# pymc-devs/pymc

Measured on AMD Instinct MI355X. Metric: effective samples/sec (and leapfrog steps/sec), 10k-param hierarchical logistic regression, one NUTS chain per GPU, higher is better.
Workload: dtype f64

## Files before the change

include/nuts_mi355.h:

```cpp
#ifndef NUTS_MI355_H
#define NUTS_MI355_H

#include <stdint.h>

#ifdef __cplusplus
extern "C" {
#endif

#define NUTS_OK 0
#define NUTS_E_BAD_ENERGY 1
#define NUTS_E_ARG 2
#define NUTS_E_HIP 3
#define NUTS_E_LINALG 4
#define NUTS_E_CALLBACK 5


enum { NUTS_TR_NONE = 0, NUTS_TR_LOG = 1, NUTS_TR_LOGODDS = 2, NUTS_TR_INTERVAL = 3 };
enum {
  NUTS_OP_CONST = 0, NUTS_OP_DATA = 1, NUTS_OP_VAR = 2,
  NUTS_OP_TMP = 3,
  NUTS_OP_GATHER = 4,
  NUTS_OP_LIN = 5
};
enum {
// ... 117 lines not shown
  const double *mix_w_const;
  const double *mix_w_alpha;
  int64_t glm_N;
  int32_t glm_P, glm_family, glm_beta, glm_intercept, glm_sigma, glm_beta_derived;
  double glm_sigma_const;
  const double *glm_X;
  const double *glm_y;
  int32_t n_lins, pad3;
  const nuts_lin *lins;
} nuts_model_spec;
enum { NUTS_GLM_NORMAL = 0, NUTS_GLM_BERNOULLI = 1, NUTS_GLM_POISSON = 2 };
#define NUTS_GLM_MAXP 512

typedef struct nuts_model nuts_model;
typedef struct nuts_chain nuts_chain;

int nuts_set_option(const char *name, int32_t value);
int nuts_unset_option(const char *name);
void nuts_clear_options(void);

int64_t nuts_edge_pair_plan(const int32_t *dirs, int32_t n_dirs, int32_t n_doublings, int32_t spec, int32_t max_depth,
                            int32_t ring, int32_t *out, int64_t out_cap);

int nuts_device_count(void);
int nuts_set_device(int device);
const char *nuts_last_error(void);

nuts_model *nuts_model_create(const nuts_model_spec *spec);
void nuts_model_destroy(nuts_model *m);
int32_t nuts_model_ndim(const nuts_model *m);
int nuts_model_logp_grad(nuts_model *m, const double *q, double *logp, double *grad);
int nuts_model_time_logp_grad(nuts_model *m, const double *q, int reps, double *ms_total, double *ms_dominant);
int nuts_model_debug_ticks(nuts_model *m, int64_t *out );
int64_t nuts_model_algorithmic_bytes(const nuts_model *m);
int nuts_model_get_scalar(const nuts_model *m, const char *name, double *out);

enum { NUTS_LL_FACTOR = 0, NUTS_LL_LOGIT_ROWS = 1, NUTS_LL_MIXTURE = 2, NUTS_LL_GLM = 3 };
int nuts_model_loglik_size(nuts_model *m, int32_t kind, int32_t index, int64_t *n);
int nuts_model_loglik(nuts_model *m, int32_t kind, int32_t index, const double *q, int64_t S, double *out);
typedef struct nuts_waic nuts_waic;
nuts_waic *nuts_waic_create(nuts_model *m, int32_t kind, int32_t index);
int nuts_waic_update(nuts_waic *w, const double *q, int64_t S);
int nuts_waic_read(nuts_waic *w, double *lppd_i, double *p_waic_i, int64_t *n_draws);
int nuts_waic_read_raw(nuts_waic *w, double *acc);
void nuts_waic_destroy(nuts_waic *w);
typedef struct nuts_psis nuts_psis;
// ... 193 lines not shown
```

pymc_amd/_lib.py:

```python

from __future__ import annotations

import ctypes as C
import os
import threading

import numpy as np

_HERE = os.path.dirname(os.path.abspath(__file__))
LIB_PATH = os.path.join(_HERE, "libnuts_mi355.so")

NUTS_OK, NUTS_E_BAD_ENERGY, NUTS_E_ARG, NUTS_E_HIP, NUTS_E_LINALG, NUTS_E_CALLBACK = 0, 1, 2, 3, 4, 5


class EngineError(RuntimeError):
    """A HIP/runtime failure inside libnuts_mi355 (maps to ParallelSamplingError-style reporting)."""


class Operand(C.Structure):
    _fields_ = [("kind", C.c_int32), ("ref", C.c_int32), ("c", C.c_double)]


class Term(C.Structure):
    _fields_ = [("a", Operand), ("b", Operand), ("c", Operand)]
# ... 215 lines not shown
    "nuts_chain_get_scalar": (C.c_int, [_VP, C.c_char_p, _PD]),
    "nuts_chain_get_vector": (C.c_int, [_VP, C.c_char_p, _PD]),
    "nuts_chain_set_dense": (C.c_int, [_VP, _PD, _PD]),
    "nuts_chain_set_diag": (C.c_int, [_VP, _PD, _PD, _PD]),
    "nuts_chain_set_host_potential": (C.c_int, [_VP, VelocityFn, EnergyFn, VelocityEnergyFn, _VP]),
    "nuts_chain_welford_export": (C.c_int, [_VP, _VP]),
    "nuts_chain_welford_import": (C.c_int, [_VP, _VP]),
    "nuts_chain_set_log_step_bar": (C.c_int, [_VP, C.c_double, C.c_double]),
    "nuts_gibbs_plan": (C.c_int, [C.POINTER(Pcg64), C.c_int64, C.c_int32, _VP, _VP, _VP, _PD]),
    "nuts_gibbs_plan_shuffle": (C.c_int, [C.POINTER(Pcg64), C.c_int64, _VP]),
    "nuts_gibbs_plan_draws": (C.c_int, [C.POINTER(Pcg64), C.c_int64, _VP, _VP, _VP, _PD, C.POINTER(C.c_int32)]),
    "nuts_gibbs_plan_skip": (C.c_int, [C.POINTER(Pcg64), C.c_int64, C.c_int32]),
    "nuts_gibbs_create": (_VP, [C.c_int64, C.c_int32, _PD]),
    "nuts_gibbs_destroy": (None, [_VP]),
    "nuts_gibbs_stage_slots": (C.c_int, []),
    "nuts_gibbs_stage": (C.c_int, [_VP, C.c_int32, _VP, _VP, _PD]),
    "nuts_gibbs_sweep_staged": (C.c_int, [_VP, C.c_int32, _VP, _VP, C.c_int32, _PD, _PD, _PD, C.POINTER(C.c_int64), C.POINTER(C.c_int64), _PD, _PD, _PD]),
    "nuts_gibbs_sweep": (C.c_int, [_VP, _VP, _PD, _PD, _PD, _VP, _VP, _PD, C.POINTER(C.c_int64), C.POINTER(C.c_int64), _PD, _PD, _PD]),
    "nuts_gibbs_plan_doubles": (C.c_int, [C.POINTER(Pcg64), C.c_int64, C.c_int32, _VP, C.c_int64, _PD]),
    "nuts_gibbs_sweep_prop": (C.c_int, [_VP, _VP, _VP, _PD, _PD, _PD, _VP, _PD, _PD, _VP, C.POINTER(C.c_int64), _PD, _PD, _PD]),
    "nuts_set_option": (C.c_int, [C.c_char_p, C.c_int32]),
    "nuts_clear_options": (None, []),
    "nuts_edge_pair_plan": (C.c_int64, [C.POINTER(C.c_int32), C.c_int32, C.c_int32, C.c_int32, C.c_int32, C.c_int32, C.POINTER(C.c_int32), C.c_int64]),
    "nuts_advi_create": (_VP, [C.POINTER(AdviConfig)]),
    "nuts_advi_destroy": (None, [_VP]),
    "nuts_advi_steps": (C.c_int, [_VP, C.c_int32, _VP, _PD, _PD]),
    "nuts_advi_get_params": (C.c_int, [_VP, _PD, _PD]),
    "nuts_advi_set_params": (C.c_int, [_VP, _PD, _PD]),
    "nuts_chain_profile": (C.c_int, [_VP, C.c_int]),
    "nuts_chain_profile_read": (C.c_int, [_VP, _PD, C.POINTER(C.c_int64), C.POINTER(C.c_int64)]),
    "nuts_group_create": (_VP, []),
    "nuts_group_add": (C.c_int, [_VP, _VP]),
    "nuts_group_remove": (C.c_int, [_VP, _VP]),
    "nuts_group_destroy": (None, [_VP]),
    "nuts_group_launches": (C.c_int, [_VP, C.POINTER(C.c_int64)]),
    "nuts_group_launches_wide": (C.c_int, [_VP, C.POINTER(C.c_int64), C.POINTER(C.c_int32)]),
    "nuts_unset_option": (C.c_int, [C.c_char_p]),
    "nuts_model_loglik_size": (C.c_int, [_VP, C.c_int32, C.c_int32, C.POINTER(C.c_int64)]),
    "nuts_model_loglik": (C.c_int, [_VP, C.c_int32, C.c_int32, _PD, C.c_int64, _PD]),
    "nuts_waic_create": (_VP, [_VP, C.c_int32, C.c_int32]),
    "nuts_waic_update": (C.c_int, [_VP, _PD, C.c_int64]),
    "nuts_waic_read": (C.c_int, [_VP, _PD, _PD, C.POINTER(C.c_int64)]),
    "nuts_waic_read_raw": (C.c_int, [_VP, _PD]),
    "nuts_waic_destroy": (None, [_VP]),
    "nuts_psis_create": (_VP, [_VP, C.c_int32, C.c_int32, C.c_int64, C.c_double]),
    "nuts_psis_update": (C.c_int, [_VP, _PD, C.c_int64]),
# ... 118 lines not shown
```

pymc_amd/csrc/engine.hip:

```cpp
#include <hip/hip_runtime.h>

#include <algorithm>
#include <atomic>
#include <chrono>
#include <cmath>
#include <cstdio>
#include <cstdlib>
#include <cstring>
#include <mutex>
#include <thread>
#include <utility>
#include <ctime>
#include <string>
#include <vector>

#include "kernels.h"
#include "small_kernel.h"
#include "mixture_kernel.h"
#include "loglik_kernel.h"
#include "predictive_kernel.h"
#include "loo_pit_kernel.h"
#include "summary_kernel.h"
#include "nuts_mi355.h"
#include "pcg64_stream.h"
// ... 2857 lines not shown
  HostStatus* st_dev = nullptr;
  HostStatus* st_host = nullptr;
  int seq = 0;
  std::vector<double> div_source, div_dest;
  bool cache_ok = false;
  std::vector<double> last_q;
  double last_logp = 0.0;
  DrawOut* do_dev = nullptr;
  DrawOut* do_host = nullptr;
  DrawOutMapped* dom_host = nullptr;
  DrawOutMapped* dom_dev = nullptr;
  unsigned dom_seq = 0;
  double* kin_part = nullptr;
  int64_t cache_epoch = -1;
  int fold_ctl = 1;
  CtlJob pend{}; bool pend_valid = false;
  bool defer_last_ctl = false; int xfold = 1;
  int next_dir = 0; bool pre_done = false; int xpre = 1;
  bool edge_pair = false;
  ArenaDev shA{};
  EdgePlan ep;
  int spec_max = 10, last_depth = 0;
  int pipe_draws = 1;
  int logs_done = 0, logs_total = 0;
  double* many_in_host = nullptr; double* many_in_dev = nullptr; char* many_out_host = nullptr; char* many_out_dev = nullptr;
  size_t many_in_cap = 0, many_out_cap = 0;
  double t_begin = 0, t_loop = 0, t_wait = 0, t_finish = 0, t_post = 0;
  double tm_pre = 0, tm_start = 0, tm_tree = 0, tm_record = 0, tm_host = 0, tm_post = 0;
  int64_t tm_draws = 0, tm_batches = 0;
  int64_t leapfrogs = 0;
  int n_uni_cap = 0;
  template <typename T>
  T* keep(T* p) { owned.push_back((void*)p); return p; }
};

extern "C" void nuts_chain_config_default(nuts_chain_config* c) {
  std::memset(c, 0, sizeof(*c));
  c->step_scale = 0.25; c->Emax = 1000; c->target_accept = 0.8; c->gamma = 0.05; c->k = 0.75; c->t0 = 10;
  c->adapt_step_size = 1; c->max_treedepth = 10; c->early_max_treedepth = 8;
  c->potential = NUTS_POT_DIAG_ADAPT; c->initial_weight = 0; c->adaptation_window = 101; c->discard_window = 50;
  c->exp_alpha = 0.02; c->exp_stop_adaptation = INFINITY; c->exp_use_grads = 0;
  c->adaptation_window_multiplier = 1; c->early_update = 0;
}

static void fa_factor(nuts_chain* c, const double* raw, double denom) {
  const int n = c->n;
// ... 154 lines not shown
  } else if (c->dense) {
    c->dense_C = c->keep(dev_upload(cfg->dense_cov, (size_t)n * n));
    c->dense_W = c->keep(dev_upload(cfg->dense_rand, (size_t)n * n));
    c->mv_grid = (n + (256 / WAVE) - 1) / (256 / WAVE);
  }
  c->n_uni_cap = (1 << maxd) + 2 * maxd + 16;
  c->stage_dev = c->keep(dev_alloc<double>(2 * (size_t)n + 2 * (size_t)c->n_uni_cap));
  c->out_dev = c->keep(dev_alloc<double>(2 * (size_t)n));
  c->out_dev2 = c->keep(dev_alloc<double>(2 * (size_t)n + 2));
  c->fold_ctl = env_int("NUTS_FOLD_CTL", 1) != 0 && !(m->md.has_mvn && m->md.mv.winv);
  c->spec_max = env_int("NUTS_SPEC_MAX", 10);
  c->xfold = env_int("NUTS_XFOLD", 1);
  c->edge_pair = m->ep_ok && env_int("NUTS_EDGE_PAIR", 1) != 0 && !c->dense && !c->host_pot && !m->md.has_mvn && !m->explicit_pre &&
                 m->md.lean_ok && c->fold_ctl && c->xfold;
  if (c->edge_pair) {
    c->shA = A;
    c->shA.S = 2;
    c->shA.Q = c->keep(dev_alloc<double>(2 * (size_t)n)); c->shA.P = c->keep(dev_alloc<double>(2 * (size_t)n));
    c->shA.V = c->keep(dev_alloc<double>(2 * (size_t)n)); c->shA.G = c->keep(dev_alloc<double>(2 * (size_t)n));
    if (!c->shA.Q || !c->shA.P || !c->shA.V || !c->shA.G) { (void)hipGetLastError(); c->edge_pair = false; }
    c->ep.ring = std::max(1, std::min(GA_RING_LEAVES, env_int("NUTS_EDGE_PAIR_RING", GA_RING_LEAVES)));
  }
  c->pipe_draws = env_int("NUTS_PIPE_DRAWS", 1) != 0;
  c->xpre = env_int("NUTS_XPRE", 1);
  c->small_lds_slots = env_int("NUTS_SMALL_LDS", 1) == 0 ? -1 : env_int("NUTS_SMALL_LDS_SLOTS", 0);
  c->small_one_wave = env_int("NUTS_SMALL_ONE_WAVE", 1);
  c->group_wide = env_int("NUTS_GROUP_WIDE", 0);
  const bool glm_small = m->md.has_glm && env_int("NUTS_GLM_SMALL", 1) != 0 && m->md.glm.Xt && !m->md.glm.beta_buf && m->md.glm.off_beta >= 0 && m->md.n_derived == 0 && n <= 256;
  c->small = env_int("NUTS_SMALL_KERNEL", 1) != 0 && n <= SMALL_MAX_N && m->ept == 1 && !m->md.has_logit && !m->md.has_mvn && !m->md.has_mix &&
             (!m->md.has_glm || glm_small) &&
             m->md.n_lins == 0 && m->factor_elems <= SMALL_MAX_ELEMS && !c->dense;
  c->do_dev = c->keep(dev_alloc<DrawOut>(1));
  A.uniforms = c->stage_dev + 2 * (size_t)n;
  A.log_uniforms = A.uniforms + c->n_uni_cap;
  for (void* p : c->owned)
    if (!p) { g_err = "device allocation failed (trajectory arena needs 4*2^max_treedepth*n*8 bytes)"; nuts_chain_destroy(c); return nullptr; }
  if (hipHostMalloc((void**)&c->stage_host, (2 * (size_t)n + 2 * (size_t)c->n_uni_cap) * sizeof(double), hipHostMallocDefault) != hipSuccess ||
      hipHostMalloc((void**)&c->out_host, 2 * (size_t)n * sizeof(double), hipHostMallocDefault) != hipSuccess ||
      hipHostMalloc((void**)&c->st_host, sizeof(HostStatus), hipHostMallocMapped) != hipSuccess ||
      hipHostGetDevicePointer((void**)&c->st_dev, c->st_host, 0) != hipSuccess ||
      hipHostMalloc((void**)&c->do_host, sizeof(DrawOut), hipHostMallocDefault) != hipSuccess ||
      hipHostMalloc((void**)&c->dom_host, DOM_RING * sizeof(DrawOutMapped), hipHostMallocMapped) != hipSuccess ||
      hipHostGetDevicePointer((void**)&c->dom_dev, c->dom_host, 0) != hipSuccess) {
    g_err = "pinned host allocation failed"; nuts_chain_destroy(c); return nullptr;
  }
  hipMemset(A.ctl, 0, sizeof(Ctl));
// ... 480 lines not shown
  HostStatus* const st = mode == MODE_TREE ? c->st_dev : (HostStatus*)nullptr;
  io.lean = m->md.lean_ok && !c->dense && (!io.explicit_pre || m->md.n_deferred == 0);
  const bool foldable = c->fold_ctl && (mode == MODE_TREE || (mode == MODE_SIMPLE && n_simple > 0));
  const bool last = mode == MODE_TREE ? j + 1 == (1 << d) : j + 1 == n_simple;
  if (io.lean && foldable) {
    if (io.explicit_pre) {
      const bool al_xpre = m->md.mv.aligned && mode == MODE_TREE && c->xpre;
      if (j == 0 && !(al_xpre && c->pre_done)) hipLaunchKernelGGL(k_leaf_pre, dim3(A.nblk), dim3(VEC_THREADS), 0, s, A, io, j);
      if (j == 0) c->pre_done = false;
      io.pre_next = last ? 0 : 1;
      if (last && al_xpre && c->defer_last_ctl && c->next_dir != 0) {
        io.pre_next = c->next_dir == gm.dir ? 1 : 3;
        c->pre_done = true;
      }
    }
    const bool deferrable = (io.explicit_pre ? m->md.mv.aligned != 0 : m->md.lg.ga != 0) && mode == MODE_TREE;
    CtlJob* job = (deferrable && j == 0 && c->pend_valid) ? &c->pend : nullptr;
    if (job && !io.explicit_pre) job->src_prev = job->io.dir == io.dir;
    launch_dense(m, A, io, j, (j > 0 || job) ? 1 : 0, d, c->cfg.Emax, max_depth, st, job);
    if (job) c->pend_valid = false;
    launch_vector(m, A, io, j, d);
    if (last) {
      if (deferrable && c->defer_last_ctl) { c->pend = CtlJob{io, j, d, seq, false}; c->pend_valid = true; }
      else launch_control_lean(m, A, io, j, d, c->cfg.Emax, max_depth, st, seq);
    }
    c->leapfrogs++;
    return;
  }
  if (io.explicit_pre) hipLaunchKernelGGL(k_leaf_pre, dim3(A.nblk), dim3(VEC_THREADS), 0, s, A, io, j);
  if (c->dense)
    dense_velocity(c, A.P + d_o, A.V + d_o, A.Q + so, A.Q + d_o, gm.eps, abort_flag, VEL_ONLY);
  launch_dense(m, A, io, j, 0, d, c->cfg.Emax, max_depth, st);
  launch_vector(m, A, io, j, d);
  if (io.lean) launch_control_lean(m, A, io, j, d, c->cfg.Emax, max_depth, st, seq);
  else if (m->has_prog) hipLaunchKernelGGL(k_control<true>, dim3(1), dim3(VEC_THREADS), 0, s, m->md, A, io, j, d, c->cfg.Emax, max_depth, st, seq);
  else hipLaunchKernelGGL(k_control<false>, dim3(1), dim3(VEC_THREADS), 0, s, m->md, A, io, j, d, c->cfg.Emax, max_depth, st, seq);
  if (c->dense) {
    dense_velocity(c, A.P + d_o, A.V + d_o, nullptr, nullptr, 0.0, abort_flag, VEL_LEAF);
    const dim3 grid(m->md.nblk);
    switch (m->ept) {
      case 1: hipLaunchKernelGGL(k_tree_vec<1>, grid, dim3(VEC_THREADS), 0, s, m->md, A, io, j, d); break;
      case 4: hipLaunchKernelGGL(k_tree_vec<4>, grid, dim3(VEC_THREADS), 0, s, m->md, A, io, j, d); break;
      default: hipLaunchKernelGGL(k_tree_vec<16>, grid, dim3(VEC_THREADS), 0, s, m->md, A, io, j, d); break;
    }
    hipLaunchKernelGGL(k_tree_ctl, dim3(1), dim3(VEC_THREADS), 0, s, m->md, A, io, j, d, c->cfg.Emax, max_depth,
                       mode == MODE_TREE ? c->st_dev : (HostStatus*)nullptr, seq);
  }
  c->leapfrogs++;
}

static int run_tree(nuts_chain* c, const double* uniforms, double step_size, int max_depth, unsigned* flags_out, bool* exhausted_out,
                    int* cursor_out = nullptr) {
  int rc = NUTS_OK;
  bool exhausted = true;
  GroupTreeScope lockstep(c->dense || c->host_pot ? nullptr : c->m);
  unsigned flags = 0;
  Geometry gm{uniforms[0] < 0.5 ? 1 : -1, 0, 0, 0, 0.0};
  gm.eps = gm.dir > 0 ? step_size : -step_size;
  auto next_geometry = [&](const Geometry& g, int d, int dir) {
    Geometry r = g;
    if (g.dir > 0) r.right += 1 << d; else r.left -= 1 << d;
    r.dir = dir;
    r.edge = dir > 0 ? r.right : r.left;
    r.eps = dir > 0 ? step_size : -step_size;
    return r;
  };
  const int spec = c->host_pot ? 0 : std::min(c->spec_max, c->last_depth - 1);
  const bool pairing = c->edge_pair && !c->m->group && !c->host_pot && !c->dense;
  int turns = 0;
  int ep_replays_in[32] = {};
  int prev_dir = 0;
  bool ep_bad = false;
  c->ep.reset();
  c->m->ep_launch.kind = EP_PLAIN;
  auto enqueue_doubling = [&](const Geometry& g, int d) {
    const int nleaf = 1 << d;
    ensure_logs(c, (2 << d) + d + 1);
    const int seq = ++c->seq;
    c->defer_last_ctl = c->xfold && c->fold_ctl && d + 1 < max_depth && d + 1 <= spec;
    c->next_dir = c->defer_last_ctl ? (uniforms[(2 << d) + d] < 0.5 ? 1 : -1) : 0;
    if (pairing) c->ep.begin(d, g.dir, std::min(spec, max_depth - 1), [&](int e) { return uniforms[(1 << e) + e - 1] < 0.5 ? 1 : -1; });
    for (int j = 0; j < nleaf; ++j) {
      if (pairing) {
        nuts_model::EpLaunch& el = c->m->ep_launch;
        int k = 0;
        el.kind = c->ep.leaf(g.dir, &el.slot, &k);
        if (el.kind == EP_REPLAY) ++ep_replays_in[std::min(d, 31)];
        if (el.kind == EP_REPLAY && k != j) { g_err = "internal error: edge pairing replays a leaf out of order"; ep_bad = true; el.kind = EP_PLAIN; }
        if (el.kind == EP_PAIRED) {
          const int od = -g.dir;
          EvalIO sio{};
          sio.mode = MODE_SIMPLE; sio.lean = 1;
          sio.dir = od; sio.edge = od > 0 ? g.right : g.left; sio.left = g.left; sio.right = g.right;
          sio.eps = od > 0 ? step_size : -step_size;
          el.sio = sio; el.sj = k; el.sA = c->shA;
          el.first = k == 0;
          el.sfold = k > 0 ? GA_FOLD_SRC : (j == 0 && d > 0 && prev_dir == od ? GA_FOLD_SRC : 0);
        }
      }
      enqueue_leaf(c, g, j, d, MODE_TREE, max_depth, j + 1 == nleaf ? seq : 0);
    }
    prev_dir = g.dir;
    c->defer_last_ctl = false;
    return seq;
  };
  c->pre_done = false;
  c->pend_valid = false;
  auto flush_pending = [&](int seq_waited) {
    if (!c->pend_valid || c->pend.seq != seq_waited) return;
    const CtlJob& p = c->pend;
    launch_control_lean(c->m, c->A, p.io, p.j, p.d, c->cfg.Emax, max_depth, c->st_dev, p.seq);
    c->pend_valid = false;
  };
  Geometry ahead{};
  int ahead_seq = 0;
  int seq = enqueue_doubling(gm, 0);
  int depth_done = 0;
  for (int d = 0; d < max_depth; ++d) {
    if (d + 1 < max_depth && d + 1 <= spec) {
      ahead = next_geometry(gm, d, uniforms[(2 << d) + d] < 0.5 ? 1 : -1);
      ahead_seq = enqueue_doubling(ahead, d + 1);
    } else ahead_seq = 0;
    flush_pending(seq);
    if (c->cb_err) return host_pot_error(c);
    const auto tw0 = clk::now();
    rc = wait_status(c, seq, &flags, cursor_out);
    c->t_wait += secs(tw0, clk::now());
    if (rc) return rc;
    depth_done = d + 1;
    if (flags & ST_BAD_ENERGY) break;
    if (flags & (ST_DIVERGING | ST_TURNING)) { exhausted = false; break; }
    if (d + 1 >= max_depth) break;
    const int dir = (flags & ST_DIR_POS) ? 1 : -1;
    turns += dir != gm.dir;
    if (ahead_seq) {
      if (ahead.dir != dir) { g_err = "internal error: look-ahead mispredicted the direction of a doubling"; return NUTS_E_HIP; }
      gm = ahead; seq = ahead_seq;
    } else {
      gm = next_geometry(gm, d, dir);
      seq = enqueue_doubling(gm, d + 1);
    }
  }
  c->last_depth = depth_done;
  c->pend_valid = false;
  if (depth_done >= 4) c->m->ep_turns = std::max(c->m->ep_turns, turns);
  c->m->ep_ring_full = c->ep.ring_full;
  if (pairing) {
    c->m->ep_dropped += c->ep.n;
    for (int d = depth_done; d < 32; ++d) c->m->ep_dropped += ep_replays_in[d];
  }
  if (ep_bad) return NUTS_E_HIP;
  *flags_out = flags;
  *exhausted_out = exhausted;
  return NUTS_OK;
}

static void launch_small(nuts_chain* c, const ArenaDev& A, const SmallDrawArgs& a) {
#define SMALL_LAUNCH(NT, P) hipLaunchKernelGGL((k_small_draw<NT, P>), dim3(1), dim3(NT), 0, c->m->stream, c->m->md, A, a)
  const bool hp = c->m->has_prog;
  if (c->n <= WAVE && c->small_one_wave && !c->m->md.has_glm) { if (hp) SMALL_LAUNCH(64, true); else SMALL_LAUNCH(64, false); }
  else if (c->n <= 256) { if (hp) SMALL_LAUNCH(256, true); else SMALL_LAUNCH(256, false); }
  else if (c->n <= 512) { if (hp) SMALL_LAUNCH(512, true); else SMALL_LAUNCH(512, false); }
  else { if (hp) SMALL_LAUNCH(1024, true); else SMALL_LAUNCH(1024, false); }
#undef SMALL_LAUNCH
}

static int finish_draw_host(nuts_chain* c, const DrawOut& o, bool adapt, bool exhausted, const double* result_dev, int64_t evals,
// ... 108 lines not shown
  double* const h_u = h_norm + (size_t)K * n;
  double* const h_lu = h_u + U;
  std::memcpy(h_q, q0, n * sizeof(double));
  std::memcpy(h_norm, normals, (size_t)K * n * sizeof(double));
  std::memcpy(h_u, uniforms, U * sizeof(double));
  for (size_t i = 0; i < U; ++i) h_lu[i] = std::log(h_u[i]);
  HIPCHK(hipMemcpyAsync(c->many_in_dev, c->many_in_host, in_doubles * sizeof(double), hipMemcpyHostToDevice, s));
  const double* const d_norm = c->many_in_dev + n;
  const double* const d_u = d_norm + (size_t)K * n;
  const double* const d_lu = d_u + U;
  double* const trace_dev = reinterpret_cast<double*>(c->many_out_dev);
  if (!cached0) {
    HIPCHK(hipMemcpyAsync(A.Q, c->many_in_dev, n * sizeof(double), hipMemcpyDeviceToDevice, s));
    model_enqueue_plain(c->m, A.Q, A.G, A.LOGP);
  }
  const double* const save_u = A.uniforms; const double* const save_lu = A.log_uniforms;
  const int save_done = c->logs_done, save_total = c->logs_total;
  c->logs_done = c->logs_total = 1 << 30;
  int done = 0;
  size_t consumed = 0;
  const int fgrid = std::max(1, std::min(256, (n + VEC_THREADS - 1) / VEC_THREADS));
  c->tm_pre += secs(tm0, clk::now()); c->tm_batches++;
  const bool pipe = !c->tune && !c->full_adapt && c->pipe_draws;
  struct Pending {
    bool valid = false; int k = 0; unsigned seq = 0; bool exhausted = false, adapt = false; size_t consumed_after = 0; int cursor = 0;
    double perf_start = 0.0, wall = 0.0, cpu = 0.0;
  } pend;
  auto enqueue_start = [&](int k, const DrawPlan& plan, size_t at, bool from_prev) {
    A.uniforms = d_u + at; A.log_uniforms = d_lu + at;
    return enqueue_draw_start(c, d_norm + (size_t)k * n, false, from_prev, plan.step_size, 0, plan.max_depth, k > 0 ? (const DrawOut*)c->do_dev : nullptr);
  };
  auto complete = [&](const Pending& p, bool* diverged) -> int {
    const auto tb = clk::now();
    DrawOutMapped* slot = c->dom_host + (p.seq % DOM_RING);
    unsigned long long seen = 0;
    int r = wait_seq(c, &slot->seq, 0, p.seq, "k_draw_finish ended without publishing its record", &seen);
    if (r) return r;
    const DrawOut o = slot->o;
    const auto t1 = clk::now();
    c->tm_record += secs(tb, t1);
    if (o.cursor != p.cursor) { g_err = "internal error: the status word and the draw record disagree on the uniforms consumed"; return NUTS_E_HIP; }
    r = finish_draw_host(c, o, p.adapt, p.exhausted, c->out_dev, o.n_proposals + ((p.k == 0 && !cached0) ? 1 : 0), p.perf_start, p.wall, p.cpu,
                         stats + p.k);
    c->tm_host += secs(t1, clk::now()); c->tm_draws++;
    if (r) return r;
    stats[p.k].n_uniforms_consumed = (int32_t)p.consumed_after;
    c->last_logp = o.logp;
    done = p.k + 1;
    *diverged = o.diverging != 0;
    return NUTS_OK;
  };
  bool started = false;
  for (int k = 0; k < K; ++k) {
    const DrawClock dclock;
    const DrawPlan plan = plan_draw(c);
    const size_t need_uni = (size_t)plan.need_uni;
    if (!started) {
      if (U - consumed < need_uni) {
        if (k == 0) { g_err = "not enough uniforms for the worst-case tree"; rc = NUTS_E_ARG; }
        break;
      }
      rc = enqueue_start(k, plan, consumed, k > 0 || cached0);
      if (rc) break;
    }
    started = false;
    unsigned flags = 0;
    bool exhausted = true;
    int cursor = 0;
    const auto ta = clk::now();
    c->tm_start += secs(dclock.t0, ta);
    rc = run_tree(c, h_u + consumed, plan.step_size, plan.max_depth, &flags, &exhausted, &cursor);
    const auto tb = clk::now();
    c->tm_tree += secs(ta, tb);
    if (rc) break;
    if (flags & ST_BAD_ENERGY) {
      if (pend.valid) { bool dv = false; rc = complete(pend, &dv); pend.valid = false; if (rc) break; }
      rc = bad_initial_energy(c);
      break;
    }
    const unsigned seq = ++c->dom_seq;
    hipLaunchKernelGGL(k_draw_finish, dim3(fgrid), dim3(VEC_THREADS), 0, s, A, c->out_dev, c->out_dev + n, c->do_dev, trace_dev + (size_t)k * n,
                       c->dom_dev + (seq % DOM_RING), seq);
    const size_t consumed_after = consumed + (size_t)cursor;
    if (pipe && !(flags & ST_DIVERGING) && k + 1 < K && U - consumed_after >= need_uni) {
      rc = enqueue_start(k + 1, plan, consumed_after, true);
      if (rc) break;
      started = true;
    }
    Pending cur;
    cur.valid = true; cur.k = k; cur.seq = seq; cur.exhausted = exhausted; cur.adapt = plan.adapt; cur.consumed_after = consumed_after; cur.cursor = cursor;
    cur.perf_start = dclock.perf_start(); cur.wall = dclock.wall(); cur.cpu = dclock.cpu();
    bool diverged = false;
    if (pend.valid) { rc = complete(pend, &diverged); pend.valid = false; if (rc) break; }
    if (started) pend = cur;
    else { rc = complete(cur, &diverged); if (rc) break; }
    consumed = consumed_after;
    if (diverged) break;
  }
  if (pend.valid) {
    bool dv = false;
    const int r2 = complete(pend, &dv);
    pend.valid = false;
    if (!rc) rc = r2;
  }
  A.uniforms = save_u; A.log_uniforms = save_lu;
  c->logs_done = save_done; c->logs_total = save_total;
  *n_done = done;
  const auto tm1 = clk::now();
  struct PostTimer { nuts_chain* c; clk::time_point t; ~PostTimer() { c->tm_post += secs(t, clk::now()); } } post_timer{c, tm1};
  if (done > 0) {
// ... 228 lines not shown
  else if (k == "tune") *out = c->tune;
  else if (k == "fg_count") *out = c->fg_count;
  else if (k == "bg_count") *out = c->bg_count;
  else if (k == "step_size") *out = c->step_size;
  else if (k == "leapfrogs") *out = (double)c->leapfrogs;
  else if (k == "tree_kernel" || k == "tree_launches") *out = 0.0;
  else if (k == "fa_fg_n") *out = c->fa_fg_n;
  else if (k == "fa_bg_n") *out = c->fa_bg_n;
  else if (k == "fa_previous_update") *out = (double)c->fa_previous_update;
  else if (k == "single_launch") *out = c->small ? 1.0 : 0.0;
  else if (k == "window_switched") *out = c->window_switched ? 1.0 : 0.0;
  else if (k == "t_begin") *out = c->t_begin;
  else if (k == "t_loop") *out = c->t_loop;
  else if (k == "t_wait") *out = c->t_wait;
  else if (k == "tm_pre") *out = c->tm_pre;
  else if (k == "tm_start") *out = c->tm_start;
  else if (k == "tm_tree") *out = c->tm_tree;
  else if (k == "tm_record") *out = c->tm_record;
  else if (k == "tm_host") *out = c->tm_host;
  else if (k == "tm_post") *out = c->tm_post;
  else if (k == "tm_draws") *out = (double)c->tm_draws;
  else if (k == "tm_batches") *out = (double)c->tm_batches;
  else if (k == "t_finish") *out = c->t_finish;
  else { g_err = "unknown scalar " + k; return NUTS_E_ARG; }
  return NUTS_OK;
}
extern "C" int nuts_chain_get_vector(nuts_chain* c, const char* name, double* out) {
  if (!c || !name || !out) return NUTS_E_ARG;
  const std::string k(name);
  const double* src = nullptr;
  if (k == "var") src = c->var;
  else if (k == "stds") src = c->stds;
  else if (k == "inv_stds") src = c->inv_stds;
  else if (k == "fg_mean") src = c->fg_is_a ? c->wa_mean : c->wb_mean;
  else if (k == "fg_m2") src = c->fg_is_a ? c->wa_m2 : c->wb_m2;
  else if (k == "bg_mean") src = c->fg_is_a ? c->wb_mean : c->wa_mean;
  else if (k == "bg_m2") src = c->fg_is_a ? c->wb_m2 : c->wa_m2;
  else if (k == "divergence_source" || k == "divergence_dest") {
    const std::vector<double>& v = k == "divergence_source" ? c->div_source : c->div_dest;
    if ((int)v.size() != c->n) { g_err = "no divergence recorded"; return NUTS_E_ARG; }
    std::memcpy(out, v.data(), c->n * sizeof(double));
    return NUTS_OK;
  }
  else if (c->full_adapt && (k == "fa_cov" || k == "fa_chol" || k == "fa_fg_raw" || k == "fa_bg_raw")) {
    src = k == "fa_cov" ? c->dense_C : k == "fa_chol" ? c->fa_L : k == "fa_fg_raw" ? c->fa_fg_raw : c->fa_bg_raw;
    HIPCHK(hipStreamSynchronize(c->m->stream));
// ... 630 lines not shown
```

pymc_amd/csrc/kernels.h:

```cpp
#pragma once
#include "model_dev.h"
#include "rows_kernel.h"

#define MAX_LEVELS 12
#define NDOT (1 + 6 * (MAX_LEVELS + 1))
#define DOT_TOP (1 + 6 * MAX_LEVELS)
#define VEC_THREADS 256
#define PART_STRIDE (PART_DOT + NDOT)

#define ROWS_BLOCK 256

#define MODE_PLAIN 0
#define MODE_TREE 1
#define MODE_SIMPLE 2

struct Ctl {
  double E0;
  double log_size, log_accept_sum, max_energy_change;
  double div_dE;
  int n_proposals, depth, left, right, proposal, cursor;
  int aborted, turning, diverging, bad_energy;
  int dir, edge;
  double eps;
  double eps_abs;
// ... 4 lines not shown
};

struct ArenaDev {
  int n, S, nblk, ept;
  double *Q, *P, *V, *G;
  double *E, *LOGP;
  double *PS;
  double *PSUM;
  const double *var, *inv_stds;
  Ctl* ctl;
  const double* uniforms;
  const double* log_uniforms;
  unsigned* ga_ticket;
  int ga_nticket;
  void* reserved;
  const double* kin_user;
};

#define ST_ABORTED 1u
#define ST_TURNING 2u
#define ST_DIVERGING 4u
#define ST_BAD_ENERGY 8u
#define ST_DIR_POS 16u
#define ST_SLOTS 4
struct HostStatus {
  unsigned long long word[ST_SLOTS];
  int aborted, turning, diverging, bad_energy, depth, cursor, n_proposals, proposal, dir, edge;
};

struct EvalIO {
  int mode;
  int explicit_pre;
  int dense;
  int lean;
  int pre_next;
  const double* q;
  double* grad;
  double* logp;
  int dir, edge;
  int left, right;
  double eps;
};

struct Leaf {
  int dir, edge, src, t, left, right;
  int64_t so, d_o;
// ... 5 lines not shown
__device__ __forceinline__ void resolve_leaf(const EvalIO& io, const ArenaDev& A, int j, Leaf& lf, QView& qv) {
  if (io.mode == MODE_PLAIN) {
    qv.q = io.q; qv.p = qv.g = qv.var = nullptr; qv.eps = qv.half = 0.0; qv.composed = 0;
    lf.dir = 1; lf.edge = lf.src = lf.t = lf.left = lf.right = 0; lf.so = lf.d_o = 0; lf.eps = lf.half = 0.0;
    return;
  }
  lf.dir = io.dir; lf.edge = io.edge; lf.left = io.left; lf.right = io.right;
  lf.src = lf.edge + lf.dir * j;
  lf.t = lf.src + lf.dir;
  lf.eps = io.eps; lf.half = 0.5 * io.eps;
  lf.so = slot_off(A, lf.src); lf.d_o = slot_off(A, lf.t);
  if (io.explicit_pre) {
    qv.q = A.Q + lf.d_o; qv.p = qv.g = qv.var = nullptr; qv.eps = qv.half = 0.0; qv.composed = 0;
  } else {
    qv.q = A.Q + lf.so; qv.p = A.P + lf.so; qv.g = A.G + lf.so; qv.var = A.var;
    qv.eps = lf.eps; qv.half = lf.half; qv.composed = 1;
  }
}

__device__ __forceinline__ int load_aborted(const EvalIO& io, const ArenaDev& A) {
  return io.mode == MODE_TREE ? __hip_atomic_load(&A.ctl->aborted, __ATOMIC_RELAXED, __HIP_MEMORY_SCOPE_AGENT) : 0;
}

__device__ __forceinline__ void publish_status(const Ctl* c, HostStatus* st, int seq) {
  if (!seq) return;
  const unsigned flags = (c->aborted ? ST_ABORTED : 0u) | (c->turning ? ST_TURNING : 0u) | (c->diverging ? ST_DIVERGING : 0u) |
                         (c->bad_energy ? ST_BAD_ENERGY : 0u) | (c->dir > 0 ? ST_DIR_POS : 0u);
  __hip_atomic_store(&st->word[seq & (ST_SLOTS - 1)],
                     ((unsigned long long)(unsigned)seq << 32) | ((unsigned long long)((unsigned)c->cursor & 0xffffffu) << 8) | flags,
                     __ATOMIC_RELAXED, __HIP_MEMORY_SCOPE_SYSTEM);
}

__device__ __forceinline__ void publish_fields(const Ctl* c, HostStatus* st) {
  st->aborted = c->aborted; st->turning = c->turning; st->diverging = c->diverging; st->bad_energy = c->bad_energy;
  st->depth = c->depth; st->cursor = c->cursor; st->n_proposals = c->n_proposals; st->proposal = c->proposal;
  st->dir = c->dir; st->edge = c->edge;
}

__global__ __launch_bounds__(VEC_THREADS) void k_leaf_pre(ArenaDev A, EvalIO io, int j) {
  if (load_aborted(io, A)) return;
  const int src = io.edge + io.dir * j, dst = src + io.dir;
  const double eps = io.eps, half = 0.5 * eps;
  const int64_t so = slot_off(A, src), d_o = slot_off(A, dst);
  const int base = blockIdx.x * VEC_THREADS * A.ept;
  for (int e = 0; e < A.ept; ++e) {
    const int i = base + e * VEC_THREADS + threadIdx.x;
    if (i < A.n) {
      const double ph = fma(half, A.G[so + i], A.P[so + i]);
      A.P[d_o + i] = ph;
      if (!io.dense) A.Q[d_o + i] = fma(eps, A.var[i] * ph, A.Q[so + i]);
// ... 1477 lines not shown
  if (blockIdx.x == 0) for (int t = threadIdx.x; t < A.ga_nticket; t += blockDim.x) A.ga_ticket[t] = 0u;
  for (int i = blockIdx.x * blockDim.x + threadIdx.x; i < A.n; i += gridDim.x * blockDim.x) {
    const double qi = A.Q[po + i];
    q_out[i] = qi;
    g_out[i] = A.G[po + i];
    if (trace_q) trace_q[i] = qi;
  }
  if (blockIdx.x == 0 && threadIdx.x == 0) {
    const int ps = prop & (A.S - 1);
    DrawOut o;
    o.energy = A.E[ps]; o.logp = A.LOGP[ps]; o.E0 = c->E0;
    o.log_accept_sum = c->log_accept_sum; o.max_energy_change = c->max_energy_change; o.div_dE = c->div_dE;
    o.depth = c->depth; o.n_proposals = c->n_proposals; o.proposal = prop; o.cursor = c->cursor;
    o.turning = c->turning; o.diverging = c->diverging; o.bad_energy = c->bad_energy; o.div_t = c->div_t;
    *out = o;
    if (mapped) {
      mapped->o = o;
      __threadfence_system();
      __hip_atomic_store(&mapped->seq, (unsigned long long)seq, __ATOMIC_RELEASE, __HIP_MEMORY_SCOPE_SYSTEM);
    }
  }
}

__global__ __launch_bounds__(VEC_THREADS) void k_potential_update(int n, const double* __restrict__ x,
                                                                  double* fg_mean, double* fg_m2, double fg_count_new,
                                                                  double* bg_mean, double* bg_m2, double bg_count_new,
                                                                  double* var, double* stds, double* inv_stds, int flags) {
  for (int i = blockIdx.x * blockDim.x + threadIdx.x; i < n; i += gridDim.x * blockDim.x) {
    double m2 = fg_m2[i];
    if (flags & 1) {
      const double xi = x[i];
      double mean = fg_mean[i];
      double od = xi - mean;
      mean += od / fg_count_new;
      m2 += od * (xi - mean);
      fg_mean[i] = mean; fg_m2[i] = m2;
      double bm = bg_mean[i], b2 = bg_m2[i];
      od = xi - bm;
      bm += od / bg_count_new;
      b2 += od * (xi - bm);
      bg_mean[i] = bm; bg_m2[i] = b2;
    }
    if (flags & 2) {
      double v = m2 / fg_count_new;
      v = fmin(fmax(v, 1e-12), 1e12);
      if (isnan(m2 / fg_count_new)) v = m2 / fg_count_new;
// ... 48 lines not shown
```

Before: 20820.

## Fuse last tree control, draw finish and next-draw start into one device kernel

Adds a k_draw_turn kernel that replaces the final control launch of a NUTS tree. When the tree is certain to end (max depth or aborted, not diverging), the same kernel writes the draw record, copies the proposal into the output buffers, and initialises momentum, energy and control state for the next draw. The host then skips the separate k_draw_finish and start launches. This removes launches and a host round-trip between draws, at the cost of a single-block kernel doing the O(n) copy and kinetic sum, plus extra host/device consistency checks.

```diff
diff --git a/include/nuts_mi355.h b/include/nuts_mi355.h
--- a/include/nuts_mi355.h
+++ b/include/nuts_mi355.h
@@ -163,6 +163,9 @@
 int64_t nuts_edge_pair_plan(const int32_t *dirs, int32_t n_dirs, int32_t n_doublings, int32_t spec, int32_t max_depth,
                             int32_t ring, int32_t *out, int64_t out_cap);
 
+int nuts_draw_turn_predicate(int32_t aborted, int32_t depth, int32_t max_depth, int32_t diverging, int32_t bad_energy,
+                             int32_t allowed, int32_t uni_left, int32_t cursor, int32_t need_uni);
+
 int nuts_device_count(void);
 int nuts_set_device(int device);
 const char *nuts_last_error(void);
diff --git a/pymc_amd/_lib.py b/pymc_amd/_lib.py
--- a/pymc_amd/_lib.py
+++ b/pymc_amd/_lib.py
@@ -261,6 +261,7 @@
     "nuts_set_option": (C.c_int, [C.c_char_p, C.c_int32]),
     "nuts_clear_options": (None, []),
     "nuts_edge_pair_plan": (C.c_int64, [C.POINTER(C.c_int32), C.c_int32, C.c_int32, C.c_int32, C.c_int32, C.c_int32, C.POINTER(C.c_int32), C.c_int64]),
+    "nuts_draw_turn_predicate": (C.c_int, [C.c_int32] * 9),
     "nuts_advi_create": (_VP, [C.POINTER(AdviConfig)]),
     "nuts_advi_destroy": (None, [_VP]),
     "nuts_advi_steps": (C.c_int, [_VP, C.c_int32, _VP, _PD, _PD]),
diff --git a/pymc_amd/csrc/engine.hip b/pymc_amd/csrc/engine.hip
--- a/pymc_amd/csrc/engine.hip
+++ b/pymc_amd/csrc/engine.hip
@@ -2903,6 +2903,11 @@
   EdgePlan ep;
   int spec_max = 10, last_depth = 0;
   int pipe_draws = 1;
+  int draw_turn = 1;
+  DrawTurn turn{};
+  bool turn_arm = false;
+  int turn_seq = 0, turn_check = 0;
+  int64_t draw_turns = 0, draw_turn_declines = 0;
   int logs_done = 0, logs_total = 0;
   double* many_in_host = nullptr; double* many_in_dev = nullptr; char* many_out_host = nullptr; char* many_out_dev = nullptr;
   size_t many_in_cap = 0, many_out_cap = 0;
@@ -3103,6 +3108,7 @@
     c->ep.ring = std::max(1, std::min(GA_RING_LEAVES, env_int("NUTS_EDGE_PAIR_RING", GA_RING_LEAVES)));
   }
   c->pipe_draws = env_int("NUTS_PIPE_DRAWS", 1) != 0;
+  c->draw_turn = env_int("NUTS_DRAW_TURN", 1) != 0;
   c->xpre = env_int("NUTS_XPRE", 1);
   c->small_lds_slots = env_int("NUTS_SMALL_LDS", 1) == 0 ? -1 : env_int("NUTS_SMALL_LDS_SLOTS", 0);
   c->small_one_wave = env_int("NUTS_SMALL_ONE_WAVE", 1);
@@ -3629,7 +3635,10 @@
     launch_vector(m, A, io, j, d);
     if (last) {
       if (deferrable && c->defer_last_ctl) { c->pend = CtlJob{io, j, d, seq, false}; c->pend_valid = true; }
-      else launch_control_lean(m, A, io, j, d, c->cfg.Emax, max_depth, st, seq);
+      else if (c->turn_arm && mode == MODE_TREE && seq && !(m->md.has_mvn && m->md.mv.aligned)) {
+        hipLaunchKernelGGL(k_draw_turn, dim3(1), dim3(VEC_THREADS), 0, s, m->md, A, io, j, d, c->cfg.Emax, max_depth, st, seq, m->ga_par, c->turn);
+        c->turn_seq = seq;
+      } else launch_control_lean(m, A, io, j, d, c->cfg.Emax, max_depth, st, seq);
     }
     c->leapfrogs++;
     return;
@@ -3654,6 +3663,11 @@
                        mode == MODE_TREE ? c->st_dev : (HostStatus*)nullptr, seq);
   }
   c->leapfrogs++;
+}
+
+extern "C" int nuts_draw_turn_predicate(int32_t aborted, int32_t depth, int32_t max_depth, int32_t diverging, int32_t bad_energy,
+                                        int32_t allowed, int32_t uni_left, int32_t cursor, int32_t need_uni) {
+  return draw_turn_ok(aborted, depth, max_depth, diverging, bad_energy, allowed, uni_left, cursor, need_uni) ? 1 : 0;
 }
 
 static int run_tree(nuts_chain* c, const double* uniforms, double step_size, int max_depth, unsigned* flags_out, bool* exhausted_out,
@@ -3686,6 +3700,7 @@
     const int seq = ++c->seq;
     c->defer_last_ctl = c->xfold && c->fold_ctl && d + 1 < max_depth && d + 1 <= spec;
     c->next_dir = c->defer_last_ctl ? (uniforms[(2 << d) + d] < 0.5 ? 1 : -1) : 0;
+    c->turn_arm = c->turn.allowed && !(d + 1 < max_depth && d + 1 <= spec);
     if (pairing) c->ep.begin(d, g.dir, std::min(spec, max_depth - 1), [&](int e) { return uniforms[(1 << e) + e - 1] < 0.5 ? 1 : -1; });
     for (int j = 0; j < nleaf; ++j) {
       if (pairing) {
@@ -3709,6 +3724,7 @@
     }
     prev_dir = g.dir;
     c->defer_last_ctl = false;
+    c->turn_arm = false;
     return seq;
   };
   c->pre_done = false;
@@ -3721,8 +3737,10 @@
   };
   Geometry ahead{};
   int ahead_seq = 0;
+  c->turn_seq = 0;
   int seq = enqueue_doubling(gm, 0);
   int depth_done = 0;
+  int cursor = 0;
   for (int d = 0; d < max_depth; ++d) {
     if (d + 1 < max_depth && d + 1 <= spec) {
       ahead = next_geometry(gm, d, uniforms[(2 << d) + d] < 0.5 ? 1 : -1);
@@ -3731,13 +3749,21 @@
     flush_pending(seq);
     if (c->cb_err) return host_pot_error(c);
     const auto tw0 = clk::now();
-    rc = wait_status(c, seq, &flags, cursor_out);
+    rc = wait_status(c, seq, &flags, &cursor);
     c->t_wait += secs(tw0, clk::now());
     if (rc) return rc;
+    if (cursor_out) *cursor_out = cursor;
+    if (c->turn_check) {
+      const unsigned long long w = *(const volatile unsigned long long*)&c->st_host->word[c->turn_check & (ST_SLOTS - 1)];
+      const bool ok = (unsigned)(w >> 32) == (unsigned)c->turn_check && ((unsigned)w & ST_TURNED);
+      c->turn_check = 0;
+      if (!ok) { g_err = "internal error: a drained turn launch did not turn the draw over"; return NUTS_E_HIP; }
+    }
     depth_done = d + 1;
     if (flags & ST_BAD_ENERGY) break;
     if (flags & (ST_DIVERGING | ST_TURNING)) { exhausted = false; break; }
     if (d + 1 >= max_depth) break;
+    if (c->turn_seq == seq) c->draw_turn_declines++;
     const int dir = (flags & ST_DIR_POS) ? 1 : -1;
     turns += dir != gm.dir;
     if (ahead_seq) {
@@ -3750,6 +3776,16 @@
   }
   c->last_depth = depth_done;
   c->pend_valid = false;
+  if (c->turn.allowed) {
+    const bool pred = nuts_draw_turn_predicate((flags & ST_ABORTED) != 0, depth_done, max_depth, (flags & ST_DIVERGING) != 0,
+                                               (flags & ST_BAD_ENERGY) != 0, c->turn.allowed, c->turn.uni_left, cursor, c->turn.need_uni) != 0;
+    if (c->turn_seq == seq) {
+      if (pred != ((flags & ST_TURNED) != 0)) { g_err = "internal error: the device's draw turn-over decision differs from the host's"; return NUTS_E_HIP; }
+    } else if (ahead_seq && c->turn_seq == ahead_seq && pred) {
+      flags |= ST_TURNED;
+      c->turn_check = ahead_seq;
+    } else if (flags & ST_TURNED) { g_err = "internal error: a draw was turned over by a launch that is not the tree's last"; return NUTS_E_HIP; }
+  }
   if (depth_done >= 4) c->m->ep_turns = std::max(c->m->ep_turns, turns);
   c->m->ep_ring_full = c->ep.ring_full;
   if (pairing) {
@@ -3904,6 +3940,8 @@
   const int fgrid = std::max(1, std::min(256, (n + VEC_THREADS - 1) / VEC_THREADS));
   c->tm_pre += secs(tm0, clk::now()); c->tm_batches++;
   const bool pipe = !c->tune && !c->full_adapt && c->pipe_draws;
+  const bool turn_cfg = c->draw_turn && !c->m->group && !c->host_pot && !c->dense && !c->m->explicit_pre && A.nblk <= DRAW_TURN_MAX_BLK;
+  c->turn_check = 0;
   struct Pending {
     bool valid = false; int k = 0; unsigned seq = 0; bool exhausted = false, adapt = false; size_t consumed_after = 0; int cursor = 0;
     double perf_start = 0.0, wall = 0.0, cpu = 0.0;
@@ -3949,9 +3987,20 @@
     unsigned flags = 0;
     bool exhausted = true;
     int cursor = 0;
+    c->turn = DrawTurn{};
+    if (turn_cfg && pipe && k + 1 < K && U - consumed <= (size_t)INT32_MAX) {
+      DrawTurn& T = c->turn;
+      T.allowed = 1; T.max_depth = plan.max_depth; T.uni_left = (int)(U - consumed); T.need_uni = plan.need_uni;
+      T.seq = c->dom_seq + 1; T.step_size = plan.step_size;
+      T.normals = d_norm + (size_t)(k + 1) * n;
+      T.q_out = c->out_dev; T.g_out = c->out_dev + n; T.trace_q = trace_dev + (size_t)k * n;
+      T.out = c->do_dev; T.mapped = c->dom_dev + (T.seq % DOM_RING);
+    }
     const auto ta = clk::now();
     c->tm_start += secs(dclock.t0, ta);
     rc = run_tree(c, h_u + consumed, plan.step_size, plan.max_depth, &flags, &exhausted, &cursor);
+    const unsigned turn_seq_given = c->turn.seq;
+    c->turn.allowed = 0;
     const auto tb = clk::now();
     c->tm_tree += secs(ta, tb);
     if (rc) break;
@@ -3961,13 +4010,20 @@
       break;
     }
     const unsigned seq = ++c->dom_seq;
-    hipLaunchKernelGGL(k_draw_finish, dim3(fgrid), dim3(VEC_THREADS), 0, s, A, c->out_dev, c->out_dev + n, c->do_dev, trace_dev + (size_t)k * n,
-                       c->dom_dev + (seq % DOM_RING), seq);
     const size_t consumed_after = consumed + (size_t)cursor;
-    if (pipe && !(flags & ST_DIVERGING) && k + 1 < K && U - consumed_after >= need_uni) {
-      rc = enqueue_start(k + 1, plan, consumed_after, true);
-      if (rc) break;
+    if (flags & ST_TURNED) {
+      if (seq != turn_seq_given) { g_err = "internal error: the draw record's sequence number moved under a turn launch"; rc = NUTS_E_HIP; break; }
+      A.uniforms = d_u + consumed_after; A.log_uniforms = d_lu + consumed_after;
+      c->draw_turns++;
       started = true;
+    } else {
+      hipLaunchKernelGGL(k_draw_finish, dim3(fgrid), dim3(VEC_THREADS), 0, s, A, c->out_dev, c->out_dev + n, c->do_dev, trace_dev + (size_t)k * n,
+                         c->dom_dev + (seq % DOM_RING), seq);
+      if (pipe && !(flags & ST_DIVERGING) && k + 1 < K && U - consumed_after >= need_uni) {
+        rc = enqueue_start(k + 1, plan, consumed_after, true);
+        if (rc) break;
+        started = true;
+      }
     }
     Pending cur;
     cur.valid = true; cur.k = k; cur.seq = seq; cur.exhausted = exhausted; cur.adapt = plan.adapt; cur.consumed_after = consumed_after; cur.cursor = cursor;
@@ -4242,6 +4298,9 @@
   else if (k == "tm_draws") *out = (double)c->tm_draws;
   else if (k == "tm_batches") *out = (double)c->tm_batches;
   else if (k == "t_finish") *out = c->t_finish;
+  else if (k == "draw_turn") *out = c->draw_turn ? 1.0 : 0.0;
+  else if (k == "draw_turns") *out = (double)c->draw_turns;
+  else if (k == "draw_turn_declines") *out = (double)c->draw_turn_declines;
   else { g_err = "unknown scalar " + k; return NUTS_E_ARG; }
   return NUTS_OK;
 }
diff --git a/pymc_amd/csrc/kernels.h b/pymc_amd/csrc/kernels.h
--- a/pymc_amd/csrc/kernels.h
+++ b/pymc_amd/csrc/kernels.h
@@ -50,6 +50,7 @@
 #define ST_DIVERGING 4u
 #define ST_BAD_ENERGY 8u
 #define ST_DIR_POS 16u
+#define ST_TURNED 32u
 #define ST_SLOTS 4
 struct HostStatus {
   unsigned long long word[ST_SLOTS];
@@ -101,10 +102,10 @@
   return io.mode == MODE_TREE ? __hip_atomic_load(&A.ctl->aborted, __ATOMIC_RELAXED, __HIP_MEMORY_SCOPE_AGENT) : 0;
 }
 
-__device__ __forceinline__ void publish_status(const Ctl* c, HostStatus* st, int seq) {
+__device__ __forceinline__ void publish_status(const Ctl* c, HostStatus* st, int seq, unsigned extra = 0u) {
   if (!seq) return;
   const unsigned flags = (c->aborted ? ST_ABORTED : 0u) | (c->turning ? ST_TURNING : 0u) | (c->diverging ? ST_DIVERGING : 0u) |
-                         (c->bad_energy ? ST_BAD_ENERGY : 0u) | (c->dir > 0 ? ST_DIR_POS : 0u);
+                         (c->bad_energy ? ST_BAD_ENERGY : 0u) | (c->dir > 0 ? ST_DIR_POS : 0u) | extra;
   __hip_atomic_store(&st->word[seq & (ST_SLOTS - 1)],
                      ((unsigned long long)(unsigned)seq << 32) | ((unsigned long long)((unsigned)c->cursor & 0xffffffu) << 8) | flags,
                      __ATOMIC_RELAXED, __HIP_MEMORY_SCOPE_SYSTEM);
@@ -1628,6 +1629,122 @@
   }
 }
 
+struct DrawTurn {
+  int allowed;
+  int max_depth, uni_left, need_uni;
+  unsigned seq;
+  double step_size;
+  const double* normals;
+  double *q_out, *g_out, *trace_q;
+  DrawOut* out;
+  DrawOutMapped* mapped;
+};
+#define DRAW_TURN_MAX_BLK 256
+
+__host__ __device__ inline bool draw_turn_ok(int aborted, int depth, int max_depth, int diverging, int bad_energy, int allowed,
+                                             int uni_left, int cursor, int need_uni) {
+  const bool over = aborted || depth >= max_depth;
+  return over && !diverging && !bad_energy && allowed && uni_left - cursor >= need_uni;
+}
+
+__global__ __launch_bounds__(VEC_THREADS) void k_draw_turn(ModelDev md, ArenaDev A, EvalIO io, int j, int d, double Emax,
+                                                          int max_depth, HostStatus* st, int seq, int par, DrawTurn T) {
+  __shared__ CtlLds lds;
+  __shared__ double s_kin[DRAW_TURN_MAX_BLK][VEC_THREADS / WAVE];
+  const int tid = threadIdx.x;
+  {
+    UniPrefetch upf;
+    uni_prefetch_none(upf);
+    control_lean_in<8, true>(md, A, io, j, d, Emax, max_depth, (HostStatus*)nullptr, 0, lean_src(md, par), 0, false, upf, lds);
+  }
+  __syncthreads();
+  const Ctl& c = lds.s_ctl;
+  const bool turn = draw_turn_ok(c.aborted, c.depth, T.max_depth, c.diverging, c.bad_energy, T.allowed && A.nblk <= DRAW_TURN_MAX_BLK,
+                                 T.uni_left, c.cursor, T.need_uni);
+  const int prop = c.proposal, final_cursor = c.cursor;
+  DrawOut o;
+  if (tid == 0) {
+    publish_status(&c, st, seq, turn ? ST_TURNED : 0u);
+    if (turn) {
+      const int ps = prop & (A.S - 1);
+      o.energy = A.E[ps]; o.logp = A.LOGP[ps]; o.E0 = c.E0;
+      o.log_accept_sum = c.log_accept_sum; o.max_energy_change = c.max_energy_change; o.div_dE = c.div_dE;
+      o.depth = c.depth; o.n_proposals = c.n_proposals; o.proposal = prop; o.cursor = final_cursor;
+      o.turning = c.turning; o.diverging = c.diverging; o.bad_energy = c.bad_energy; o.div_t = c.div_t;
+    }
+  }
+  if (!turn) return;
+  for (int t = tid; t < A.ga_nticket; t += VEC_THREADS) A.ga_ticket[t] = 0u;
+  if (tid == 0) {
+    *T.out = o;
+    T.mapped->o = o;
+    __threadfence_system();
+    __hip_atomic_store(&T.mapped->seq, (unsigned long long)T.seq, __ATOMIC_RELEASE, __HIP_MEMORY_SCOPE_SYSTEM);
+  }
+  const int64_t po = slot_off(A, prop);
+  const int lane = tid & (WAVE - 1), w = tid >> 6;
+  constexpr int U = 16;
+  const int nrow = A.nblk * A.ept;
+  double kin = 0.0;
+  for (int k0 = 0; k0 < nrow; k0 += U) {
+    double q[U], g[U], z[U], is[U], vr[U];
+#pragma unroll
+    for (int u = 0; u < U; ++u) {
+      const int i = (k0 + u) * VEC_THREADS + tid;
+      const int ii = (k0 + u < nrow && i < A.n) ? i : 0;
+      q[u] = A.Q[po + ii]; g[u] = A.G[po + ii]; z[u] = T.normals[ii]; is[u] = A.inv_stds[ii]; vr[u] = A.var[ii];
+    }
+#pragma unroll
+    for (int u = 0; u < U; ++u) {
+      const int k = k0 + u;
+      if (k >= nrow) break;
+      const int i = k * VEC_THREADS + tid;
+      if (i < A.n) {
+        T.q_out[i] = q[u]; T.g_out[i] = g[u];
+        if (T.trace_q) T.trace_q[i] = q[u];
+        const double p = z[u] * is[u];
+        const double v = vr[u] * p;
+        A.P[i] = p; A.V[i] = v; A.PSUM[i] = p;
+        A.Q[i] = q[u]; A.G[i] = g[u];
+        kin = fma(p, v, kin);
+      }
+      if ((k + 1) % A.ept == 0) {
+        const double tot = wave_sum(kin);
+        if (lane == 0) s_kin[k / A.ept][w] = tot;
+        kin = 0.0;
+      }
+    }
+  }
+  __syncthreads();
+  for (int b = tid; b < A.nblk; b += VEC_THREADS) {
+    double r = 0.0;
+    for (int i = 0; i < VEC_THREADS / WAVE; ++i) r += s_kin[b][i];
+    s_kin[b][0] = r;
+  }
+  __syncthreads();
+  if (tid != 0) return;
+  double s = 0.0;
+  for (int b = 0; b < A.nblk; ++b) s += s_kin[b][0];
+  Ctl* cn = A.ctl;
+  A.LOGP[0] = o.logp;
+  const double E = 0.5 * s - o.logp;
+  A.E[0] = E;
+  cn->E0 = E;
+  cn->log_size = 0.0;
+  cn->log_accept_sum = -INFINITY;
+  cn->max_energy_change = 0.0;
+  cn->div_dE = 0.0;
+  cn->n_proposals = 0; cn->depth = 0; cn->left = 0; cn->right = 0; cn->proposal = 0; cn->cursor = 0;
+  cn->turning = 0; cn->diverging = 0;
+  cn->bad_energy = !isfinite(E);
+  cn->aborted = cn->bad_energy;
+  cn->eps_abs = T.step_size;
+  cn->n_leaves_total = 0;
+  cn->dir = 1; cn->edge = 0; cn->eps = T.step_size;
+  if (!cn->aborted && T.max_depth > 0) ctl_next_direction(cn, A.uniforms + final_cursor);
+  publish_fields(cn, st);
+}
+
 __global__ __launch_bounds__(VEC_THREADS) void k_potential_update(int n, const double* __restrict__ x,
                                                                   double* fg_mean, double* fg_m2, double fg_count_new,
                                                                   double* bg_mean, double* bg_m2, double bg_count_new,
```

Result: no change. 20810, median of 2 (-0.0%).
